# cg-saarland/hagrid

Hardware: AMD Instinct MI355X
Metric: Mrays/s (primary traversal) + grid build ms, 1M-tri scene @1/2/4/8 MI355X (higher is better)
Workload: dtype f32

## Files before the change

### hagrid_amd/csrc/ctx.h

```cpp
#pragma once

#include <hip/hip_runtime.h>

#include <atomic>
#include <cstdio>
#include <memory>
#include <string>
#include <unordered_map>
#include <vector>

#include "hagrid_amd.h"

namespace hagrid_impl {

struct Slot {
    void* ptr = nullptr;
    size_t size = 0;
    bool in_use = false;
    int refs = 0;
};

}

namespace hagrid_impl {

struct TravImageCache {
    void* table = nullptr;
    size_t table_bytes = 0;
    int wide_records = 0;
    void* blocks = nullptr;
    size_t block_bytes = 0;
    bool valid = false;
    bool uniform = false;
    bool general = false;
    int slim = 0;
    int vtop_k = 0;
    uint32_t vtop_base = 0;
    bool detached = false;
    bool borrowed = false;
    std::shared_ptr<std::atomic<bool>> alive;
    const void* entries = nullptr; const void* cells = nullptr; const void* refs = nullptr;
    int num_cells = 0, num_entries = 0, num_refs = 0, shift = 0, dims[3] = {0, 0, 0}, cell_bytes = 32;
    int max_ref = -1;
    void* alt_blocks = nullptr; void* alt_table = nullptr; size_t alt_block_bytes = 0, alt_table_bytes = 0; int alt_wide_records = 0, alt_slim = 0;
};

}

namespace hagrid_impl {
enum MailboxWord : int {
    kMbxRowLen = 300,
    kMbxOrderStale = 304,
    kMbxReadBackEpoch = 310,
    kMbxHeadSuggest = 312,
    kMbxPriorStats = 316,
};
enum ScratchWord : int {
    kScrRowLenBinned = 232,
    kScrRowLen = 236,
    kScrMaxRef = 240,
    kScrBlobFlag = 250,
};
}

struct hagrid_ctx {
    int device = 0;
    hipStream_t stream = nullptr;
    bool keep = false;
    int num_cus = 0;

    std::vector<hagrid_impl::Slot> slots;
    std::unordered_map<void*, int> tracker;
    size_t usage = 0, max_usage = 0;

    hipEvent_t ev_begin = nullptr, ev_end = nullptr;

    int* mailbox = nullptr;
    int* dscratch = nullptr;
    unsigned long long* lb_state = nullptr;
    size_t lb_words = 0;
    unsigned lb_epoch = 0;
    int* row_scores = nullptr;
    int* bin_diff = nullptr;

    int ray_binning = 0;
    int opt_variant = 0;
    int opt_lookback = 1;
    int opt_merge_inplace = 1;
    int opt_merge_inplace_iters = 0;
    int opt_merge_inplace_div = 0;
    int opt_merge_inplace_room = 0;
    int opt_merge_narrow = 1;
    int opt_expand_voxel_map = 1;
    int opt_expand_subset_only = 1;
    int opt_image_width = 0;
    int opt_band_rows = 0;
    int opt_super_log2 = 3;
    int opt_xcd_chunk_log2 = -2;
    int opt_narrow = 1;
    int opt_image_max_mb = 0;
    int opt_quad_head = 20;
    int opt_image_vtop = 1;
    int opt_image_uniform = 1;
    int opt_row_cache = 1;
    struct RayHints {
        const void* key_rays = nullptr; int key_n = 0;
        const void* rowlen_rays = nullptr; int rowlen_n = 0, rowlen_age = 0, rowlen_known = -1, rowlen_seen = 0; bool rows_from_origins = false ;
        hipEvent_t rowlen_evt = nullptr; bool rowlen_pending = false;
        int* lpt_buf = nullptr; int lpt_cap = 0; const void* lpt_rays = nullptr; int lpt_n = 0, lpt_blocks = 0, lpt_age = 0, lpt_period = 32, lpt_rot = 0 ; bool rot_adopted = false ;
        hipEvent_t trial_evt[2] = {nullptr, nullptr}; bool trial_pending = false, trial_with_head = false, head_disabled = false;
        float t_base = 0.0f, t_head = 0.0f; int n_base = 0, n_head = 0, trial_opt = -1 ; unsigned head_serial = 0 ; bool lpt_valid = false;
        int lpt_epoch = 1 , relearn_streak = 0, cooldown = 0, cooldown_len = 64; unsigned long long relearn_clock = 0;
        hipEvent_t share_evt[12][2] = {}; int share_issued = 0, share_done = 0, share_choice = -1 , share_ncand = 0 , share_shape_nc = 0 , share_cands[4] = {0, 0, 0, 0} ,
            share_last = -1 , share_launches = 0; float share_t[4] = {0.0f, 0.0f, 0.0f, 0.0f}; unsigned share_serial = 0 ;
        int trial_kind = 0 , n_all = 0, all_stage = 0 ; float t_all = 0.0f; bool learned_all = false;
        bool learned_once = false;
        unsigned order_serial = 0;
        bool cmp_pending = false, cmp_done = false; int n_conf = 0; float t_conf = 0.0f;
        bool order_loses = false;
        int last_report = -1;
        unsigned long long used = 0;
    };
    static constexpr int kRayHints = 4;
    RayHints hints[kRayHints];
    unsigned long long hint_clock = 0;
    int opt_mailbox = -1;
    int opt_tail = 1;
    int opt_lds_pad = 0;
    int opt_tail_dual = -1;
    int opt_share_trial = 1;
    int opt_order_gate = 1;
    int opt_tile_order = -1;
    int opt_quad_tail = -1;
    int opt_image_slim = 1;
    int opt_image_general = 1;
    int opt_image = 2;

    int opt_id_is_steps = 0;

    hagrid_impl::TravImageCache image;
    unsigned image_serial = 0;
    int readback_epoch = 0;
    int opt_fast_readback = 1;
    int build_arena_tris = 0;
    size_t build_arena_hint = 0;
    hagrid_build_counts counts = {};

    std::string err;
};

namespace hagrid_impl {

inline int fail(hagrid_ctx* ctx, int code, const char* file, int line, const char* msg) {
    if (ctx) {
        char buf[512];
        snprintf(buf, sizeof(buf), "%s(%d): %s", file, line, msg);
        ctx->err = buf;
    }
    return code;
}

#define HG_FAIL(ctx, code, msg) return ::hagrid_impl::fail((ctx), (code), __FILE__, __LINE__, (msg))
#define HG_HIP(ctx, call)                                                                         \
    do {                                                                                          \
        hipError_t e_ = (call);                                                                   \
        if (e_ != hipSuccess) return ::hagrid_impl::fail((ctx), HAGRID_EHIP, __FILE__, __LINE__, hipGetErrorString(e_)); \
    } while (0)
#define HG_TRY(expr)                                                                              \
    do {                                                                                          \
        int rc_ = (expr);                                                                         \
        if (rc_ < 0) return rc_;                                                                  \
    } while (0)

void debug_sync(hagrid_ctx* ctx, const char* file, int line);
#ifdef HAGRID_DEBUG_SYNC
#define HG_DBG(ctx) ::hagrid_impl::debug_sync((ctx), __FILE__, __LINE__)
#else
#define HG_DBG(ctx) do { } while (0)
#endif

template <typename T>
inline T* pool_alloc(hagrid_ctx* ctx, size_t n) {
    return static_cast<T*>(hagrid_mem_alloc(ctx, (n ? n : 1) * sizeof(T)));
}

template <typename T>
inline T* pool_try_alloc(hagrid_ctx* ctx, size_t n) {
    const std::string saved = ctx->err;
    T* p = pool_alloc<T>(ctx, n);
    if (!p) { (void)hipGetLastError(); ctx->err = saved; }
    return p;
}

struct PoolTemps {
    hagrid_ctx* ctx;
    std::vector<void*> ptrs;
    explicit PoolTemps(hagrid_ctx* c) : ctx(c) {}
    PoolTemps(const PoolTemps&) = delete;
    PoolTemps& operator=(const PoolTemps&) = delete;
    template <typename T> T* get(size_t n) { T* p = pool_alloc<T>(ctx, n); if (p) ptrs.push_back(p); return p; }
    void drop(void* p) { for (auto& q : ptrs) if (q == p && p) { hagrid_mem_free(ctx, p); q = nullptr; } }
    void* keep(void* p) { for (auto& q : ptrs) if (q == p) q = nullptr; return p; }
    ~PoolTemps() { for (void* p : ptrs) if (p) hagrid_mem_free(ctx, p); }
};

int pool_split(hagrid_ctx* ctx, void* base, void* const* parts, int n);

int read_back(hagrid_ctx* ctx, const void* dptr, void* hptr, size_t bytes);

inline int grid_blocks(long long n, int block) { return (int)((n + block - 1) / block); }

unsigned long long* lookback_state(hagrid_ctx* ctx, int tiles, int words_per_tile, unsigned* epoch);

int trav_image_build(hagrid_ctx* ctx, const hagrid_grid* grid);
void trav_image_drop(hagrid_ctx* ctx);
bool trav_image_matches(const hagrid_ctx* ctx, const hagrid_grid* grid);
bool trav_image_stale(const hagrid_ctx* ctx);
void trav_image_source_touched(hagrid_ctx* ctx, const void* ptr, size_t bytes);

}
```

### hagrid_amd/csrc/expand.hip

```cpp
#include "ctx.h"
#include "wave_prims.h"

#include "hagrid/grid.h"
#include "hagrid/prims.h"

using namespace hagrid;
using namespace hagrid_impl;

namespace {

struct ExpandK { ivec3 dims; ivec3 top; int shift; vec3 gmin, cell_size, grid_inv; const int* voxel_cells; };
constexpr int kChanged = 1 << 3;
struct CellRec { ivec3 lo; int begin; ivec3 hi; int end; };

__device__ __forceinline__ CellRec load_cell(const Cell* cells, int i) {
    const int4* p = reinterpret_cast<const int4*>(cells) + 2 * size_t(i);
    const int4 a = p[0], b = p[1];
    CellRec c; c.lo = ivec3(a.x, a.y, a.z); c.begin = a.w; c.hi = ivec3(b.x, b.y, b.z); c.end = b.w;
    return c;
}
__device__ __forceinline__ int comp(const ivec3& v, int axis) { return axis == 0 ? v.x : (axis == 1 ? v.y : v.z); }


__device__ __forceinline__ int lower_bound_in(const int* __restrict__ a, int n, int x) {
    int lo = 0, hi = n;
    while (lo < hi) {
        const int mid = (lo + hi) >> 1;
        if (a[mid] < x) lo = mid + 1; else hi = mid;
    }
    return lo;
}

__device__ __forceinline__ bool contains_all(const int* __restrict__ big, int nbig, const int* __restrict__ small, int nsmall) {
    if (nsmall > nbig) return false;
    if (nsmall == 0) return true;
    if (nbig <= 4) {
        const int b0 = big[0], b1 = nbig > 1 ? big[1] : -1, b2 = nbig > 2 ? big[2] : -1, b3 = nbig > 3 ? big[3] : -1;
        const int s0 = small[0], s1 = nsmall > 1 ? small[1] : s0, s2 = nsmall > 2 ? small[2] : s0, s3 = nsmall > 3 ? small[3] : s0;
        auto in_big = [&](int x) { return (x == b0) | (x == b1) | (x == b2) | (x == b3); };
        return in_big(s0) & in_big(s1) & in_big(s2) & in_big(s3);
    }
    for (int j = 0; j < nsmall; j++) {
        const int x = small[j], at = lower_bound_in(big, nbig, x);
        if (at == nbig || big[at] != x) return false;
    }
    return true;
}

__device__ __forceinline__ Tri load_tri(const float4* __restrict__ tris, int i) {
    const float4* p = tris + 3 * size_t(i);
    const float4 a = p[0], b = p[1], c = p[2];
    return Tri(vec3(a.x, a.y, a.z), a.w, vec3(b.x, b.y, b.z), b.w, vec3(c.x, c.y, c.z), c.w);
}

__global__ void __launch_bounds__(kBlock) fill_voxel_cells(ExpandK k, const Entry* __restrict__ entries, int* __restrict__ voxel_cells, int voxels) {
    const int v = blockIdx.x * kBlock + threadIdx.x;
    if (v >= voxels) return;
    const int s = k.shift, m = (1 << s) - 1, top = v >> (3 * s), local = v & ((1 << (3 * s)) - 1);
    const int tx = top % k.top.x, ty = (top / k.top.x) % k.top.y, tz = top / (k.top.x * k.top.y);
    const ivec3 at((tx << s) + (local & m), (ty << s) + ((local >> s) & m), (tz << s) + (local >> (2 * s)));
    voxel_cells[v] = int(lookup_entry(entries, s, k.top, at));
}
__device__ __forceinline__ int cell_of_voxel(const ExpandK& k, const Entry* __restrict__ entries, const ivec3& at) {
    if (!k.voxel_cells) return int(lookup_entry(entries, k.shift, k.top, at));
    const int s = k.shift, m = (1 << s) - 1;
    const int top = (at.x >> s) + k.top.x * ((at.y >> s) + k.top.y * (at.z >> s));
    return k.voxel_cells[(top << (3 * s)) + (at.x & m) + (((at.y & m) + ((at.z & m) << s)) << s)];
}

template <int AXIS>
__device__ __forceinline__ int room_before_prim(const ExpandK& k, const Tri& prim, const CellRec& cell, const BBox& cross, int room, bool UP) {
    constexpr int A1 = (AXIS + 1) % 3, A2 = (AXIS + 2) % 3;
    const BBox pb = prim.bbox();
    const bool overlaps = get<A1>(pb.min) <= get<A1>(cross.max) && get<A1>(pb.max) >= get<A1>(cross.min) &&
                          get<A2>(pb.min) <= get<A2>(cross.max) && get<A2>(pb.max) >= get<A2>(cross.min);
    if (!overlaps) return room;
    const int layer = int(((UP ? get<AXIS>(pb.min) : get<AXIS>(pb.max)) - get<AXIS>(k.gmin)) * get<AXIS>(k.grid_inv));
    const int free_layers = UP ? layer - comp(cell.hi, AXIS) : comp(cell.lo, AXIS) - layer - 1;
    return max(min(room, free_layers), 0);
}

template <int AXIS, bool SUBSET_ONLY>
__device__ __forceinline__ int face_growth(const ExpandK& k, const Entry* __restrict__ entries, const int* __restrict__ refs, const float4* __restrict__ tris,
                                           const Cell* __restrict__ cells, const CellRec& cell, bool UP, bool& again) {
    constexpr int A1 = (AXIS + 1) % 3, A2 = (AXIS + 2) % 3;
    const int face = UP ? comp(cell.hi, AXIS) : comp(cell.lo, AXIS);
    const int extent = comp(k.dims, AXIS);
    if (UP ? face >= extent : face <= 0) return 0;
    const int layer = UP ? face : face - 1;
    const int lo1 = comp(cell.lo, A1), hi1 = comp(cell.hi, A1), lo2 = comp(cell.lo, A2), hi2 = comp(cell.hi, A2);
    const int own = cell.end - cell.begin;
    int reach = extent, room = extent;
    int u = lo1, v = lo2, row_step = comp(k.dims, A2);
    for (;;) {
        const ivec3 at = AXIS == 0 ? ivec3(layer, u, v) : (AXIS == 1 ? ivec3(v, layer, u) : ivec3(u, v, layer));
        const CellRec nb = load_cell(cells, cell_of_voxel(k, entries, at));
        reach = min(reach, UP ? comp(nb.hi, AXIS) - face : face - comp(nb.lo, AXIS));
        room = min(room, reach);
        const int theirs = nb.end - nb.begin;
        if (SUBSET_ONLY) {
            if (!contains_all(refs + cell.begin, own, refs + nb.begin, theirs)) { room = 0; break; }
        } else if (theirs > 0) {
            const BBox cross(k.gmin + k.cell_size * vec3(cell.lo), k.gmin + k.cell_size * vec3(cell.hi));
            int mine = 0;
            for (int j = 0; j < theirs && room > 0; j++) {
                const int id = refs[nb.begin + j];
                while (mine < own && refs[cell.begin + mine] < id) mine++;
                if (mine < own && refs[cell.begin + mine] == id) continue;
                room = room_before_prim<AXIS>(k, load_tri(tris, id), cell, cross, room, UP);
            }
            if (room == 0) break;
        }
        row_step = min(row_step, comp(nb.hi, A2) - v);
        u = comp(nb.hi, A1);
        if (u >= hi1) {
            u = lo1; v += row_step; row_step = comp(k.dims, A2);
            if (v >= hi2) break;
        }
    }
    again |= room == reach;
    return UP ? room : -room;
}

template <int axis, bool SUBSET_ONLY, bool PAIRED>
__device__ __forceinline__ void grow_cell(const ExpandK& k, const Entry* __restrict__ entries, const int* __restrict__ refs, const float4* __restrict__ tris,
                                          const Cell* __restrict__ cells, Cell* __restrict__ new_cells, unsigned char* __restrict__ cell_flags, int id, int flags, bool up) {
    CellRec cell = load_cell(cells, id);
    bool flag = false;
    int ov1, ov2;
    if (PAIRED) {
        bool again = false;
        const int mine = face_growth<axis, SUBSET_ONLY>(k, entries, refs, tris, cells, cell, up, again);
        const int other = __shfl_xor(mine, 1, 64);
        flag = again | (__shfl_xor(int(again), 1, 64) != 0);
        if (up) return;
        ov1 = mine; ov2 = other;
    } else {
        ov1 = face_growth<axis, SUBSET_ONLY>(k, entries, refs, tris, cells, cell, false, flag);
        ov2 = face_growth<axis, SUBSET_ONLY>(k, entries, refs, tris, cells, cell, true, flag);
    }
    if (axis == 0) { cell.lo.x += ov1; cell.hi.x += ov2; }
    if (axis == 1) { cell.lo.y += ov1; cell.hi.y += ov2; }
    if (axis == 2) { cell.lo.z += ov1; cell.hi.z += ov2; }
    cell_flags[id] = (unsigned char)((flag ? 1 << axis : 0) | (flags & ~((1 << axis) | kChanged)) | ((ov1 | ov2) ? kChanged : 0));
    int4* out = reinterpret_cast<int4*>(new_cells) + 2 * size_t(id);
    out[0] = make_int4(cell.lo.x, cell.lo.y, cell.lo.z, cell.begin);
    out[1] = make_int4(cell.hi.x, cell.hi.y, cell.hi.z, cell.end);
}

template <int axis, bool SUBSET_ONLY>
__global__ void __launch_bounds__(kBlock) overlap_step(ExpandK k, const Entry* __restrict__ entries, const int* __restrict__ refs,
                                                       const float4* __restrict__ tris, const Cell* __restrict__ cells, Cell* __restrict__ new_cells,
                                                       unsigned char* __restrict__ cell_flags, int num_cells) {
    const int id = xcd_block(blockIdx.x, gridDim.x) * kBlock + threadIdx.x;
    if (id >= num_cells) return;
    const int flags = cell_flags[id];
    if ((flags & (1 << axis)) == 0) {
        const int4* p = reinterpret_cast<const int4*>(cells) + 2 * size_t(id);
        int4* out = reinterpret_cast<int4*>(new_cells) + 2 * size_t(id);
        const int4 a = p[0], b = p[1];
        out[0] = a; out[1] = b;
        if (flags & kChanged) cell_flags[id] = (unsigned char)(flags & ~kChanged);
        return;
    }
    grow_cell<axis, SUBSET_ONLY, false>(k, entries, refs, tris, cells, new_cells, cell_flags, id, flags, false);
}

constexpr int kSelectItems = 16;
constexpr int kSelectTile = kBlock * kSelectItems;

template <int axis>
__global__ void __launch_bounds__(kBlock) expand_select(const Cell* __restrict__ cells, Cell* __restrict__ new_cells, unsigned char* __restrict__ cell_flags,
                                                        int num_cells, int* __restrict__ list, int* __restrict__ count) {
    __shared__ int tile_list[kSelectTile];
    __shared__ int tile_count, tile_base;
    if (threadIdx.x == 0) tile_count = 0;
    __syncthreads();
    const int base = blockIdx.x * kSelectTile;
    int fl[kSelectItems];
    #pragma unroll
    for (int j = 0; j < kSelectItems; j++) {
        const int id = base + j * kBlock + threadIdx.x;
        fl[j] = id < num_cells ? cell_flags[id] : 0;
    }
    #pragma unroll
    for (int j = 0; j < kSelectItems; j++) {
        const int id = base + j * kBlock + threadIdx.x;
        const int flags = fl[j];
        const bool listed = (flags & (1 << axis)) != 0;
        const unsigned long long m = __ballot(listed);
        int wbase = 0;
        if (lane_id() == 0 && m) wbase = atomicAdd(&tile_count, __popcll(m));
        wbase = __shfl(wbase, 0, 64);
        if (listed) {
            tile_list[wbase + __popcll(m & ((1ull << lane_id()) - 1ull))] = id;
        } else if (flags & kChanged) {
            const int4* p = reinterpret_cast<const int4*>(cells) + 2 * size_t(id);
            int4* out = reinterpret_cast<int4*>(new_cells) + 2 * size_t(id);
            const int4 a = p[0], b = p[1];
            out[0] = a; out[1] = b;
            cell_flags[id] = (unsigned char)(flags & ~kChanged);
        }
    }
    __syncthreads();
    if (threadIdx.x == 0) tile_base = tile_count ? atomicAdd(count, tile_count) : 0;
    __syncthreads();
    for (int i = threadIdx.x; i < tile_count; i += kBlock) list[tile_base + i] = tile_list[i];
}

template <int axis, bool SUBSET_ONLY>
__global__ void __launch_bounds__(kBlock) expand_listed(ExpandK k, const Entry* __restrict__ entries, const int* __restrict__ refs,
                                                        const float4* __restrict__ tris, const Cell* __restrict__ cells, Cell* __restrict__ new_cells,
                                                        unsigned char* __restrict__ cell_flags, const int* __restrict__ list, const int* __restrict__ count) {
    const int n = *count, active = (2 * n + kBlock - 1) / kBlock;
    if (int(blockIdx.x) >= active) return;
    const int t = xcd_block(blockIdx.x, active) * kBlock + threadIdx.x;
    const int i = t >> 1;
    if (i >= n) return;
    const int id = list[i];
    grow_cell<axis, SUBSET_ONLY, true>(k, entries, refs, tris, cells, new_cells, cell_flags, id, cell_flags[id], (t & 1) != 0);
}

template <int axis, bool SUBSET_ONLY>
void listed_step(hipStream_t st, const ExpandK& k, const Entry* entries, const int* refs, const float4* tris, const Cell* cells, Cell* other,
                 unsigned char* flags, int n, int* list, int* count) {
    expand_select<axis><<<grid_blocks(n, kSelectTile), kBlock, 0, st>>>(cells, other, flags, n, list, count);
    expand_listed<axis, SUBSET_ONLY><<<grid_blocks(2ll * n, kBlock), kBlock, 0, st>>>(k, entries, refs, tris, cells, other, flags, list, count);
}

}

extern "C" int hagrid_expand_grid(hagrid_ctx* ctx, hagrid_grid* grid, const void* tris_v, int iters) {
    if (!ctx || !grid) return HAGRID_EINVAL;
    const bool subset_only = ctx->opt_expand_subset_only != 0;
    if (!subset_only && !tris_v && iters > 0) HG_FAIL(ctx, HAGRID_EINVAL, "expand_grid: the precise mode needs the triangles");
    const float4* tris = static_cast<const float4*>(tris_v);
    if (iters <= 0) return HAGRID_OK;
    if (!grid->cells || !grid->entries || !grid->ref_ids) HG_FAIL(ctx, HAGRID_EINVAL, "expand_grid: incomplete (or compressed) grid");
    trav_image_drop(ctx);
    HG_HIP(ctx, hipSetDevice(ctx->device));
    hipStream_t st = ctx->stream;
    ExpandK k;
    k.top = ivec3(grid->dims[0], grid->dims[1], grid->dims[2]);
    k.dims = k.top << grid->shift;
    k.shift = grid->shift;
    {
        const vec3 lo(grid->bbox_min[0], grid->bbox_min[1], grid->bbox_min[2]), ext = vec3(grid->bbox_max[0], grid->bbox_max[1], grid->bbox_max[2]) - lo;
        k.gmin = lo; k.cell_size = ext / vec3(k.dims); k.grid_inv = vec3(k.dims) / ext;
    }
    const int n = grid->num_cells;
    Cell* cells = static_cast<Cell*>(grid->cells);
    Cell* other = pool_alloc<Cell>(ctx, size_t(n));
    unsigned char* flags = pool_alloc<unsigned char>(ctx, size_t(n));
    if (!other || !flags) { hagrid_mem_free(ctx, other); hagrid_mem_free(ctx, flags); return HAGRID_ENOMEM; }
    (void)hipMemsetAsync(flags, 0xFF, size_t(n), st);
    const Entry* entries = static_cast<const Entry*>(grid->entries);
    const int* refs = static_cast<const int*>(grid->ref_ids);
    const int blocks = grid_blocks(n, kBlock);
    int* list = iters > 1 ? pool_try_alloc<int>(ctx, size_t(n)) : nullptr;
    const long long voxels = (long long)k.dims.x * k.dims.y * k.dims.z;
    int* voxel_cells = (ctx->opt_expand_voxel_map && voxels <= (1ll << 28)) ? pool_try_alloc<int>(ctx, size_t(voxels)) : nullptr;
    k.voxel_cells = voxel_cells;
    if (voxel_cells) { ExpandK kf = k; kf.voxel_cells = nullptr; fill_voxel_cells<<<grid_blocks(voxels, kBlock), kBlock, 0, st>>>(kf, entries, voxel_cells, int(voxels)); HG_DBG(ctx); }
    int* counts = ctx->dscratch + 160;
    const int max_listed = 48;
    if (list) (void)hipMemsetAsync(counts, 0, max_listed * sizeof(int), st);
    int listed = 0;
    for (int it = 0; it < iters; it++) {
        if (it > 0 && list && listed + 3 <= max_listed) {
            if (subset_only) {
                listed_step<0, true>(st, k, entries, refs, tris, cells, other, flags, n, list, counts + listed++); std::swap(cells, other);
                listed_step<1, true>(st, k, entries, refs, tris, cells, other, flags, n, list, counts + listed++); std::swap(cells, other);
                listed_step<2, true>(st, k, entries, refs, tris, cells, other, flags, n, list, counts + listed++); std::swap(cells, other);
            } else {
                listed_step<0, false>(st, k, entries, refs, tris, cells, other, flags, n, list, counts + listed++); std::swap(cells, other);
                listed_step<1, false>(st, k, entries, refs, tris, cells, other, flags, n, list, counts + listed++); std::swap(cells, other);
                listed_step<2, false>(st, k, entries, refs, tris, cells, other, flags, n, list, counts + listed++); std::swap(cells, other);
            }
            continue;
        }
        if (subset_only) {
            overlap_step<0, true><<<blocks, kBlock, 0, st>>>(k, entries, refs, tris, cells, other, flags, n); HG_DBG(ctx); std::swap(cells, other);
            overlap_step<1, true><<<blocks, kBlock, 0, st>>>(k, entries, refs, tris, cells, other, flags, n); HG_DBG(ctx); std::swap(cells, other);
            overlap_step<2, true><<<blocks, kBlock, 0, st>>>(k, entries, refs, tris, cells, other, flags, n); HG_DBG(ctx); std::swap(cells, other);
        } else {
            overlap_step<0, false><<<blocks, kBlock, 0, st>>>(k, entries, refs, tris, cells, other, flags, n); HG_DBG(ctx); std::swap(cells, other);
            overlap_step<1, false><<<blocks, kBlock, 0, st>>>(k, entries, refs, tris, cells, other, flags, n); HG_DBG(ctx); std::swap(cells, other);
            overlap_step<2, false><<<blocks, kBlock, 0, st>>>(k, entries, refs, tris, cells, other, flags, n); HG_DBG(ctx); std::swap(cells, other);
        }
    }
    hipError_t e = hipGetLastError();
    if (e == hipSuccess) e = hipStreamSynchronize(st);
    ctx->counts.expand_passes = 3 * iters; ctx->counts.expand_cells = n;
    hagrid_mem_free(ctx, flags);
    hagrid_mem_free(ctx, other);
    hagrid_mem_free(ctx, list);
    hagrid_mem_free(ctx, voxel_cells);
    grid->cells = cells;
    if (e != hipSuccess) HG_FAIL(ctx, HAGRID_EHIP, hipGetErrorString(e));
    return HAGRID_OK;
}
```

### hagrid_amd/csrc/kat/kat.hip

```cpp
#include "../trav_kernels.h"
#include "hagrid_amd_kat.h"

#include <cstring>

using namespace hagrid;
using namespace hagrid_impl;
using namespace hagrid_trav;


namespace {

__global__ void kat_prim_ray(const Tri* tris, const Ray* rays, const int* idx, int n, int* ret, int* hid, float* ht) {
    const int i = blockIdx.x * blockDim.x + threadIdx.x;
    if (i >= n) return;
    Hit h(-1, rays[i].tmax, 0, 0);
    ret[i] = intersect_prim_ray(tris[idx[i]], rays[i], idx[i], h) ? 1 : 0;
    hid[i] = h.id; ht[i] = h.t;
}
__global__ void kat_prim_ray_uvs(const Tri* tris, const Ray* rays, const int* idx, int n, int* ret, int* hid, float* ht, float* hu, float* hv) {
    const int i = blockIdx.x * blockDim.x + threadIdx.x;
    if (i >= n) return;
    Hit h(-1, rays[i].tmax, 0, 0);
    ret[i] = intersect_prim_ray_uvs(tris[idx[i]], rays[i], idx[i], h) ? 1 : 0;
    hid[i] = h.id; ht[i] = h.t; hu[i] = h.u; hv[i] = h.v;
// ... 95 lines not shown
                o[4 + j] = id == none ? ~0u : id;
                if (id != none) cnt++;
            }
            o[3] = cnt | (links ? 0x40000000u : 0u);
        }
        return;
    }
}

struct Staged {
    hagrid_ctx* ctx; void* d = nullptr; size_t bytes;
    Staged(hagrid_ctx* c, const void* h, size_t b) : ctx(c), bytes(b) {
        d = hagrid_mem_alloc(ctx, b);
        if (d && h) hagrid_mem_copy_h2d(ctx, d, h, b);
    }
    ~Staged() { hagrid_mem_free(ctx, d); }
    int fetch(void* h) { return hagrid_mem_copy_d2h(ctx, h, d, bytes); }
};

}

extern "C" int hagrid_kat_intersect_prim_ray(hagrid_ctx* ctx, const void* tris, const void* rays, const int32_t* tri_index,
                                             int n, int32_t* ret, int32_t* hit_id, float* hit_t) {
    if (!ctx || n <= 0) return HAGRID_EINVAL;
    int max_idx = 0;
    for (int i = 0; i < n; i++) max_idx = std::max(max_idx, tri_index[i]);
    Staged t(ctx, tris, size_t(max_idx + 1) * 48), r(ctx, rays, size_t(n) * 32), ix(ctx, tri_index, size_t(n) * 4);
    Staged o0(ctx, nullptr, size_t(n) * 4), o1(ctx, nullptr, size_t(n) * 4), o2(ctx, nullptr, size_t(n) * 4);
    kat_prim_ray<<<grid_blocks(n, 64), 64, 0, ctx->stream>>>((const Tri*)t.d, (const Ray*)r.d, (const int*)ix.d, n, (int*)o0.d, (int*)o1.d, (float*)o2.d); HG_DBG(ctx);
    HG_HIP(ctx, hipGetLastError());
    HG_TRY(o0.fetch(ret)); HG_TRY(o1.fetch(hit_id)); HG_TRY(o2.fetch(hit_t));
    return HAGRID_OK;
}

extern "C" int hagrid_kat_intersect_prim_ray_uvs(hagrid_ctx* ctx, const void* tris, const void* rays, const int32_t* tri_index,
                                                 int n, int32_t* ret, int32_t* hit_id, float* hit_t, float* hit_u, float* hit_v) {
    if (!ctx || n <= 0) return HAGRID_EINVAL;
    int max_idx = 0;
    for (int i = 0; i < n; i++) max_idx = std::max(max_idx, tri_index[i]);
    Staged t(ctx, tris, size_t(max_idx + 1) * 48), r(ctx, rays, size_t(n) * 32), ix(ctx, tri_index, size_t(n) * 4);
    Staged o0(ctx, nullptr, size_t(n) * 4), o1(ctx, nullptr, size_t(n) * 4), o2(ctx, nullptr, size_t(n) * 4), o3(ctx, nullptr, size_t(n) * 4), o4(ctx, nullptr, size_t(n) * 4);
    kat_prim_ray_uvs<<<grid_blocks(n, 64), 64, 0, ctx->stream>>>((const Tri*)t.d, (const Ray*)r.d, (const int*)ix.d, n, (int*)o0.d, (int*)o1.d, (float*)o2.d, (float*)o3.d, (float*)o4.d); HG_DBG(ctx);
    HG_HIP(ctx, hipGetLastError());
    HG_TRY(o0.fetch(ret)); HG_TRY(o1.fetch(hit_id)); HG_TRY(o2.fetch(hit_t)); HG_TRY(o3.fetch(hit_u)); HG_TRY(o4.fetch(hit_v));
    return HAGRID_OK;
}

extern "C" int hagrid_kat_intersect_prim_cell(hagrid_ctx* ctx, const void* tris, const void* boxes, const int32_t* tri_index, int n, int32_t* ret) {
    if (!ctx || n <= 0) return HAGRID_EINVAL;
    int max_idx = 0;
    for (int i = 0; i < n; i++) max_idx = std::max(max_idx, tri_index[i]);
    Staged t(ctx, tris, size_t(max_idx + 1) * 48), b(ctx, boxes, size_t(n) * 32), ix(ctx, tri_index, size_t(n) * 4), o(ctx, nullptr, size_t(n) * 4);
    kat_prim_cell<<<grid_blocks(n, 64), 64, 0, ctx->stream>>>((const Tri*)t.d, (const BBox*)b.d, (const int*)ix.d, n, (int*)o.d); HG_DBG(ctx);
    HG_HIP(ctx, hipGetLastError());
    return o.fetch(ret);
}

extern "C" int hagrid_kat_compute_range(hagrid_ctx* ctx, const int32_t* dims3, const void* grid_bb, const void* obj_bb, int n, int32_t* out6) {
    if (!ctx || n <= 0) return HAGRID_EINVAL;
    Staged d(ctx, dims3, size_t(n) * 12), g(ctx, grid_bb, size_t(n) * 32), ob(ctx, obj_bb, size_t(n) * 32), o(ctx, nullptr, size_t(n) * 24);
    kat_range<<<grid_blocks(n, 64), 64, 0, ctx->stream>>>((const int*)d.d, (const BBox*)g.d, (const BBox*)ob.d, n, (int*)o.d); HG_DBG(ctx);
    HG_HIP(ctx, hipGetLastError());
    return o.fetch(out6);
}

extern "C" int hagrid_kat_compute_grid_dims(hagrid_ctx* ctx, const void* bb, const int32_t* num_prims, const float* density, int n, int32_t* out3) {
    if (!ctx || n <= 0) return HAGRID_EINVAL;
    Staged b(ctx, bb, size_t(n) * 32), np(ctx, num_prims, size_t(n) * 4), de(ctx, density, size_t(n) * 4), o(ctx, nullptr, size_t(n) * 12);
    kat_grid_dims<<<grid_blocks(n, 64), 64, 0, ctx->stream>>>((const BBox*)b.d, (const int*)np.d, (const float*)de.d, n, (int*)o.d); HG_DBG(ctx);
    HG_HIP(ctx, hipGetLastError());
    return o.fetch(out3);
}

extern "C" int hagrid_kat_lookup_entry(hagrid_ctx* ctx, const uint32_t* entries, int num_entries, int shift, const int32_t* top_dims3,
                                       const int32_t* voxels3, int n, uint32_t* out) {
    if (!ctx || n <= 0 || num_entries <= 0) return HAGRID_EINVAL;
    Staged e(ctx, entries, size_t(num_entries) * 4), v(ctx, voxels3, size_t(n) * 12), o(ctx, nullptr, size_t(n) * 4);
    kat_lookup<<<grid_blocks(n, 64), 64, 0, ctx->stream>>>((const Entry*)e.d, shift, ivec3(top_dims3[0], top_dims3[1], top_dims3[2]), (const int*)v.d, n, (uint32_t*)o.d); HG_DBG(ctx);
    HG_HIP(ctx, hipGetLastError());
    return o.fetch(out);
}

extern "C" int hagrid_kat_detect_ray_rows(hagrid_ctx* ctx, const void* rays_dev, int num_rays, float bbox_diag, int32_t* row_len) {
    if (!ctx || !rays_dev || num_rays < 0 || !row_len) return HAGRID_EINVAL;
    int* d = ctx->dscratch + 232;
    TraverseArgs a;
    memset(&a, 0, sizeof(a));
    a.rays = static_cast<const float4*>(rays_dev);
    a.max_x = bbox_diag; a.min_x = 0.0f;
    launch_detect(ctx, a, num_rays, d, 65536);
    HG_HIP(ctx, hipGetLastError());
    HG_TRY(read_back(ctx, d, row_len, sizeof(int)));
    *row_len &= kRowLenMask;
    return HAGRID_OK;
}

extern "C" int hagrid_kat_tile_slots(hagrid_ctx* ctx, int num_rays, int row_len, int super_log2, int xcd_chunk_log2, int32_t* slots) {
    if (!ctx || num_rays <= 0 || !slots || super_log2 < 0 || (super_log2 & 0xff) > 8) return HAGRID_EINVAL;
    const int blocks = grid_blocks(num_rays, 64);
    TraverseArgs a;
    memset(&a, 0, sizeof(a));
    a.num_rays = num_rays; a.row_len_hint = row_len; a.super_log2 = super_log2 & 0xff; a.band_rows = super_log2 >> 8; a.xcd_chunk_log2 = xcd_chunk_log2;
    Staged o(ctx, nullptr, size_t(blocks) * 64 * 4);
    if (!o.d) return HAGRID_ENOMEM;
    kat_tile_slots<<<blocks, 64, 0, ctx->stream>>>(a, (int*)o.d); HG_DBG(ctx);
    HG_HIP(ctx, hipGetLastError());
    return o.fetch(slots);
}

extern "C" int hagrid_kat_image_records(hagrid_ctx* ctx, const hagrid_grid* grid, const int32_t* voxels3, int n, uint32_t* records8, int64_t* image_bytes) {
    if (!ctx || !grid || n < 0) return HAGRID_EINVAL;
    if (!trav_image_matches(ctx, grid)) HG_FAIL(ctx, HAGRID_EINVAL, "no traversal image for this grid");
    if (image_bytes) *image_bytes = (int64_t)ctx->image.block_bytes + (int64_t)ctx->image.table_bytes;
    if (n == 0) return HAGRID_OK;
    TraverseArgs a;
    HG_TRY(make_args(ctx, grid, nullptr, nullptr, nullptr, 0, a));
    image_args(ctx, a);
    Staged v(ctx, voxels3, size_t(n) * 12), o(ctx, nullptr, size_t(n) * 32);
    if (!v.d || !o.d) return HAGRID_ENOMEM;
    kat_image_records<<<grid_blocks(n, 64), 64, 0, ctx->stream>>>(a, (const int*)v.d, n, (uint32_t*)o.d, 1, ctx->image.slim, ctx->image.uniform ? 1 : 0, ctx->image.general ? 1 : 0); HG_DBG(ctx);
    HG_HIP(ctx, hipGetLastError());
    return o.fetch(records8);
}

extern "C" int hagrid_kat_traverse_timed(hagrid_ctx* ctx, const hagrid_grid* grid, const void* tris, const void* rays, void* hits, int num_rays,
                                         int row_len, int tail, unsigned long long* times_dev, const int* tile_order_dev) {
    if (!ctx || !grid || !times_dev || num_rays <= 0) return HAGRID_EINVAL;
    if (!trav_image_matches(ctx, grid) || !(ctx->image.uniform && ctx->image.slim == 20))
        HG_FAIL(ctx, HAGRID_EINVAL, "kat_traverse_timed: needs the table-free image with 20-bit slim records of this grid");
    TraverseArgs a;
    HG_TRY(make_args(ctx, grid, tris, rays, hits, num_rays, a));
    image_args(ctx, a);
    a.row_len_hint = row_len; a.wave_times = times_dev; a.tile_order = tile_order_dev;
    const int blocks = grid_blocks(num_rays, 64);
    if (tail) traverse_kernel_tail<20, true><<<blocks, 64, 0, ctx->stream>>>(a);
    else      traverse_kernel_img<0, 20, 0, true><<<blocks, 64, 0, ctx->stream>>>(a);
    HG_DBG(ctx);
    HG_HIP(ctx, hipGetLastError());
    return HAGRID_OK;
}

extern "C" int hagrid_kat_set_option(hagrid_ctx* ctx, const char* key, int value) {
    if (!ctx || !key) return HAGRID_EINVAL;
    struct { const char* name; int* dst; int lo, hi; } table[] = {
        {"traverse.variant", &ctx->opt_variant, 0, 4},              {"traverse.narrow", &ctx->opt_narrow, 0, 1},
        {"traverse.image_uniform", &ctx->opt_image_uniform, 0, 2},  {"traverse.image_slim", &ctx->opt_image_slim, 1, 2}, {"traverse.image_general", &ctx->opt_image_general, 0, 2}, {"traverse.image_vtop", &ctx->opt_image_vtop, 0, 1}, {"traverse.quad_head", &ctx->opt_quad_head, 0, 1000}, {"ctx.fast_readback", &ctx->opt_fast_readback, 0, 1},
        {"traverse.tail", &ctx->opt_tail, 0, 1},                    {"traverse.quad_tail", &ctx->opt_quad_tail, -1, 100},
        {"traverse.tail_dual", &ctx->opt_tail_dual, -1, 1},        
        {"traverse.super_tile", &ctx->opt_super_log2, 0, 8},        {"traverse.xcd_chunk", &ctx->opt_xcd_chunk_log2, -2, 16},
        {"traverse.row_cache", &ctx->opt_row_cache, 0, 1},          {"traverse.lds_pad", &ctx->opt_lds_pad, 0, 65536},
        {"merge.narrow_cells", &ctx->opt_merge_narrow, 0, 1},       {"scan.lookback", &ctx->opt_lookback, 1, 2},
        {"traverse.order_gate", &ctx->opt_order_gate, 0, 1}, {"traverse.share_trial", &ctx->opt_share_trial, 0, 1}, {"traverse.band_rows", &ctx->opt_band_rows, 0, 1 << 16}, {"traverse.mailbox", &ctx->opt_mailbox, -1, 1},
        {"merge.inplace", &ctx->opt_merge_inplace, 0, 1},           {"merge.inplace_iters", &ctx->opt_merge_inplace_iters, 0, 1 << 20}, {"merge.inplace_room", &ctx->opt_merge_inplace_room, 0, 0x7fffffff}, {"merge.inplace_div", &ctx->opt_merge_inplace_div, 0, 1 << 20},
        {"expand.voxel_map", &ctx->opt_expand_voxel_map, 0, 1},
    };
    for (auto& t : table)
        if (!strcmp(key, t.name)) {
            if (value < t.lo || value > t.hi || (t.dst == &ctx->opt_variant && value == 3)) HG_FAIL(ctx, HAGRID_EINVAL, "kat_set_option: value out of range");
            *t.dst = value;
            return HAGRID_OK;
        }
    return hagrid_set_option(ctx, key, value);
}

extern "C" int hagrid_kat_order_state(hagrid_ctx* ctx, const void* rays, int32_t* out12, float* ms2 ) {
    if (!ctx || !out12) return HAGRID_EINVAL;
    for (int i = 0; i < 12; i++) out12[i] = 0;
    out12[0] = -1;
    for (int i = 0; i < hagrid_ctx::kRayHints; i++) {
        const hagrid_ctx::RayHints& h = ctx->hints[i];
        if (h.key_rays != rays) continue;
        const int v[12] = {i, h.lpt_valid, h.cooldown > 0, h.lpt_rot, h.head_disabled, h.n_base, h.n_head, h.share_choice >= 0 ? h.share_cands[h.share_choice] : -1, h.share_done + 100 * h.share_issued + 10000 * int(h.order_loses), h.n_all + 10 * int(h.learned_all) + 100 * h.cooldown, __atomic_load_n(ctx->mailbox + kMbxHeadSuggest + i, __ATOMIC_RELAXED), h.share_launches};
        for (int k = 0; k < 12; k++) out12[k] = v[k];
        if (ms2) { ms2[0] = h.t_base; ms2[1] = h.t_head; ms2[2] = h.t_all; ms2[3] = h.share_choice >= 0 ? h.share_t[h.share_choice] : 0.0f; }
        return HAGRID_OK;
    }
    return HAGRID_OK;
}

extern "C" int hagrid_kat_forget_hints(hagrid_ctx* ctx) {
    if (!ctx) return HAGRID_EINVAL;
    for (auto& h : ctx->hints) { h.key_rays = nullptr; h.key_n = 0; h.used = 0; h.lpt_rays = nullptr; h.lpt_valid = false; h.rowlen_rays = nullptr; h.rowlen_seen = 0; h.share_ncand = 0; h.share_shape_nc = 0; h.share_choice = -1; }
    return HAGRID_OK;
}
```

Before: 7712.

## Use packed 16-byte narrow cell records with inline ref lists during grid expansion

```diff
diff --git a/hagrid_amd/csrc/ctx.h b/hagrid_amd/csrc/ctx.h
--- a/hagrid_amd/csrc/ctx.h
+++ b/hagrid_amd/csrc/ctx.h
@@ -92,6 +92,7 @@
     int opt_merge_inplace_room = 0;
     int opt_merge_narrow = 1;
     int opt_expand_voxel_map = 1;
+    int opt_expand_narrow = 1;
     int opt_expand_subset_only = 1;
     int opt_image_width = 0;
     int opt_band_rows = 0;
diff --git a/hagrid_amd/csrc/expand.hip b/hagrid_amd/csrc/expand.hip
--- a/hagrid_amd/csrc/expand.hip
+++ b/hagrid_amd/csrc/expand.hip
@@ -9,15 +9,56 @@
 
 namespace {
 
-struct ExpandK { ivec3 dims; ivec3 top; int shift; vec3 gmin, cell_size, grid_inv; const int* voxel_cells; };
+struct ExpandK {
+    ivec3 dims; ivec3 top; int shift; vec3 gmin, cell_size, grid_inv;
+    const int* voxel_cells;
+    const Cell* orig;
+    int subset_only;
+};
 constexpr int kChanged = 1 << 3;
+constexpr int kGrew = 1 << 4;
 struct CellRec { ivec3 lo; int begin; ivec3 hi; int end; };
 
-__device__ __forceinline__ CellRec load_cell(const Cell* cells, int i) {
-    const int4* p = reinterpret_cast<const int4*>(cells) + 2 * size_t(i);
-    const int4 a = p[0], b = p[1];
-    CellRec c; c.lo = ivec3(a.x, a.y, a.z); c.begin = a.w; c.hi = ivec3(b.x, b.y, b.z); c.end = b.w;
+constexpr int kListShift = 29;
+constexpr uint32_t kPayload = (1u << kListShift) - 1u;
+constexpr int kLong = 7;
+
+template <bool NARROW>
+__device__ __forceinline__ CellRec load_cell(const void* cells, int i) {
+    CellRec c;
+    if (NARROW) {
+        const uint4 v = reinterpret_cast<const uint4*>(cells)[i];
+        c.lo = ivec3(int(v.x & 0xffffu), int(v.x >> 16), int(v.y & 0xffffu));
+        c.hi = ivec3(int(v.y >> 16), int(v.z & 0xffffu), int(v.z >> 16));
+        c.begin = int(v.w); c.end = 0;
+    } else {
+        const int4* p = reinterpret_cast<const int4*>(cells) + 2 * size_t(i);
+        const int4 a = p[0], b = p[1];
+        c.lo = ivec3(a.x, a.y, a.z); c.begin = a.w; c.hi = ivec3(b.x, b.y, b.z); c.end = b.w;
+    }
     return c;
+}
+template <bool NARROW>
+__device__ __forceinline__ void store_cell(void* cells, int i, const CellRec& c) {
+    if (NARROW) {
+        reinterpret_cast<uint4*>(cells)[i] = make_uint4(uint32_t(c.lo.x) | uint32_t(c.lo.y) << 16, uint32_t(c.lo.z) | uint32_t(c.hi.x) << 16,
+                                                        uint32_t(c.hi.y) | uint32_t(c.hi.z) << 16, uint32_t(c.begin));
+    } else {
+        int4* out = reinterpret_cast<int4*>(cells) + 2 * size_t(i);
+        out[0] = make_int4(c.lo.x, c.lo.y, c.lo.z, c.begin);
+        out[1] = make_int4(c.hi.x, c.hi.y, c.hi.z, c.end);
+    }
+}
+template <bool NARROW>
+__device__ __forceinline__ void copy_cell(const void* cells, void* new_cells, int i) {
+    if (NARROW) {
+        reinterpret_cast<uint4*>(new_cells)[i] = reinterpret_cast<const uint4*>(cells)[i];
+    } else {
+        const int4* p = reinterpret_cast<const int4*>(cells) + 2 * size_t(i);
+        int4* out = reinterpret_cast<int4*>(new_cells) + 2 * size_t(i);
+        const int4 a = p[0], b = p[1];
+        out[0] = a; out[1] = b;
+    }
 }
 __device__ __forceinline__ int comp(const ivec3& v, int axis) { return axis == 0 ? v.x : (axis == 1 ? v.y : v.z); }
 
@@ -47,19 +88,59 @@
     return true;
 }
 
+struct ListRef { int n, at, one; };
+__device__ __forceinline__ ListRef list_of(const ExpandK& k, uint32_t word, int cell) {
+    const int count = int(word >> kListShift), pay = int(word & kPayload);
+    ListRef l; l.at = pay; l.one = pay;
+    l.n = count == kLong ? reinterpret_cast<const int*>(k.orig)[8 * size_t(cell) + 7] - pay : count;
+    return l;
+}
+
+struct OwnList {
+    int n, b0, b1, b2, b3; const int* p;
+    __device__ __forceinline__ bool has(int x) const {
+        if (n <= 4) return (x == b0) | (x == b1) | (x == b2) | (x == b3);
+        const int at = lower_bound_in(p, n, x);
+        return at < n && p[at] == x;
+    }
+};
+__device__ __forceinline__ OwnList own_list(const ExpandK& k, const int* __restrict__ refs, uint32_t word, int cell) {
+    const ListRef l = list_of(k, word, cell);
+    const bool inline_id = (word >> kListShift) == 1u;
+    const bool regs = !inline_id && l.n <= 4;
+    OwnList o; o.n = l.n; o.p = refs + l.at;
+    o.b0 = inline_id ? l.one : (regs && l.n > 0 ? o.p[0] : -1);
+    o.b1 = regs && l.n > 1 ? o.p[1] : -1; o.b2 = regs && l.n > 2 ? o.p[2] : -1; o.b3 = regs && l.n > 3 ? o.p[3] : -1;
+    return o;
+}
+__device__ __forceinline__ bool own_contains(const ExpandK& k, const int* __restrict__ refs, const OwnList& own, uint32_t word, int nb) {
+    const int count = int(word >> kListShift);
+    if (count == 0) return true;
+    if (own.n == 0) return false;
+    if (count == 1) return own.has(int(word & kPayload));
+    const ListRef l = list_of(k, word, nb);
+    if (l.n > own.n) return false;
+    const int* small = refs + l.at;
+    if (own.n <= 4) {
+        const int s0 = small[0], s1 = l.n > 1 ? small[1] : s0, s2 = l.n > 2 ? small[2] : s0, s3 = l.n > 3 ? small[3] : s0;
+        return own.has(s0) & own.has(s1) & own.has(s2) & own.has(s3);
+    }
+    for (int j = 0; j < l.n; j++)
+        if (!own.has(small[j])) return false;
+    return true;
+}
+
 __device__ __forceinline__ Tri load_tri(const float4* __restrict__ tris, int i) {
     const float4* p = tris + 3 * size_t(i);
     const float4 a = p[0], b = p[1], c = p[2];
     return Tri(vec3(a.x, a.y, a.z), a.w, vec3(b.x, b.y, b.z), b.w, vec3(c.x, c.y, c.z), c.w);
 }
 
-__global__ void __launch_bounds__(kBlock) fill_voxel_cells(ExpandK k, const Entry* __restrict__ entries, int* __restrict__ voxel_cells, int voxels) {
-    const int v = blockIdx.x * kBlock + threadIdx.x;
-    if (v >= voxels) return;
+__device__ __forceinline__ int voxel_cell(const ExpandK& k, const Entry* __restrict__ entries, int v) {
     const int s = k.shift, m = (1 << s) - 1, top = v >> (3 * s), local = v & ((1 << (3 * s)) - 1);
     const int tx = top % k.top.x, ty = (top / k.top.x) % k.top.y, tz = top / (k.top.x * k.top.y);
     const ivec3 at((tx << s) + (local & m), (ty << s) + ((local >> s) & m), (tz << s) + (local >> (2 * s)));
-    voxel_cells[v] = int(lookup_entry(entries, s, k.top, at));
+    return int(lookup_entry(entries, s, k.top, at));
 }
 __device__ __forceinline__ int cell_of_voxel(const ExpandK& k, const Entry* __restrict__ entries, const ivec3& at) {
     if (!k.voxel_cells) return int(lookup_entry(entries, k.shift, k.top, at));
@@ -80,10 +161,14 @@
     return max(min(room, free_layers), 0);
 }
 
-template <int AXIS, bool SUBSET_ONLY>
+template <int MODE> __device__ __forceinline__ bool subset_mode(const ExpandK& k) { return MODE == 0 ? k.subset_only != 0 : MODE == 1; }
+
+template <int AXIS, int MODE>
 __device__ __forceinline__ int face_growth(const ExpandK& k, const Entry* __restrict__ entries, const int* __restrict__ refs, const float4* __restrict__ tris,
-                                           const Cell* __restrict__ cells, const CellRec& cell, bool UP, bool& again) {
+                                           const void* __restrict__ cells, const CellRec& cell, const OwnList& mine_list, bool UP, bool& again) {
     constexpr int A1 = (AXIS + 1) % 3, A2 = (AXIS + 2) % 3;
+    constexpr bool NARROW = MODE != 0;
+    const bool subset_only = subset_mode<MODE>(k);
     const int face = UP ? comp(cell.hi, AXIS) : comp(cell.lo, AXIS);
     const int extent = comp(k.dims, AXIS);
     if (UP ? face >= extent : face <= 0) return 0;
@@ -94,13 +179,29 @@
     int u = lo1, v = lo2, row_step = comp(k.dims, A2);
     for (;;) {
         const ivec3 at = AXIS == 0 ? ivec3(layer, u, v) : (AXIS == 1 ? ivec3(v, layer, u) : ivec3(u, v, layer));
-        const CellRec nb = load_cell(cells, cell_of_voxel(k, entries, at));
+        const int nb_id = cell_of_voxel(k, entries, at);
+        const CellRec nb = load_cell<NARROW>(cells, nb_id);
         reach = min(reach, UP ? comp(nb.hi, AXIS) - face : face - comp(nb.lo, AXIS));
         room = min(room, reach);
-        const int theirs = nb.end - nb.begin;
-        if (SUBSET_ONLY) {
-            if (!contains_all(refs + cell.begin, own, refs + nb.begin, theirs)) { room = 0; break; }
-        } else if (theirs > 0) {
+        if (subset_only) {
+            const bool sub = NARROW ? own_contains(k, refs, mine_list, uint32_t(nb.begin), nb_id)
+                                    : contains_all(refs + cell.begin, own, refs + nb.begin, nb.end - nb.begin);
+            if (!sub) { room = 0; break; }
+        } else if (NARROW) {
+            const int count = int(uint32_t(nb.begin) >> kListShift);
+            if (count > 0) {
+                const ListRef l = list_of(k, uint32_t(nb.begin), nb_id);
+                const BBox cross(k.gmin + k.cell_size * vec3(cell.lo), k.gmin + k.cell_size * vec3(cell.hi));
+                for (int j = 0; j < l.n && room > 0; j++) {
+                    int id = l.one;
+                    if (count != 1) id = refs[l.at + j];
+                    if (mine_list.has(id)) continue;
+                    room = room_before_prim<AXIS>(k, load_tri(tris, id), cell, cross, room, UP);
+                }
+                if (room == 0) break;
+            }
+        } else if (nb.end - nb.begin > 0) {
+            const int theirs = nb.end - nb.begin;
             const BBox cross(k.gmin + k.cell_size * vec3(cell.lo), k.gmin + k.cell_size * vec3(cell.hi));
             int mine = 0;
             for (int j = 0; j < theirs && room > 0; j++) {
@@ -122,55 +223,53 @@
     return UP ? room : -room;
 }
 
-template <int axis, bool SUBSET_ONLY, bool PAIRED>
+template <int axis, int MODE, bool PAIRED>
 __device__ __forceinline__ void grow_cell(const ExpandK& k, const Entry* __restrict__ entries, const int* __restrict__ refs, const float4* __restrict__ tris,
-                                          const Cell* __restrict__ cells, Cell* __restrict__ new_cells, unsigned char* __restrict__ cell_flags, int id, int flags, bool up) {
-    CellRec cell = load_cell(cells, id);
+                                          const void* __restrict__ cells, void* __restrict__ new_cells, unsigned char* __restrict__ cell_flags, int id, int flags, bool up) {
+    constexpr bool NARROW = MODE != 0;
+    CellRec cell = load_cell<NARROW>(cells, id);
+    OwnList own = {};
+    if (NARROW) own = own_list(k, refs, uint32_t(cell.begin), id);
     bool flag = false;
     int ov1, ov2;
     if (PAIRED) {
         bool again = false;
-        const int mine = face_growth<axis, SUBSET_ONLY>(k, entries, refs, tris, cells, cell, up, again);
+        const int mine = face_growth<axis, MODE>(k, entries, refs, tris, cells, cell, own, up, again);
         const int other = __shfl_xor(mine, 1, 64);
         flag = again | (__shfl_xor(int(again), 1, 64) != 0);
         if (up) return;
         ov1 = mine; ov2 = other;
     } else {
-        ov1 = face_growth<axis, SUBSET_ONLY>(k, entries, refs, tris, cells, cell, false, flag);
-        ov2 = face_growth<axis, SUBSET_ONLY>(k, entries, refs, tris, cells, cell, true, flag);
+        ov1 = face_growth<axis, MODE>(k, entries, refs, tris, cells, cell, own, false, flag);
+        ov2 = face_growth<axis, MODE>(k, entries, refs, tris, cells, cell, own, true, flag);
     }
     if (axis == 0) { cell.lo.x += ov1; cell.hi.x += ov2; }
     if (axis == 1) { cell.lo.y += ov1; cell.hi.y += ov2; }
     if (axis == 2) { cell.lo.z += ov1; cell.hi.z += ov2; }
-    cell_flags[id] = (unsigned char)((flag ? 1 << axis : 0) | (flags & ~((1 << axis) | kChanged)) | ((ov1 | ov2) ? kChanged : 0));
-    int4* out = reinterpret_cast<int4*>(new_cells) + 2 * size_t(id);
-    out[0] = make_int4(cell.lo.x, cell.lo.y, cell.lo.z, cell.begin);
-    out[1] = make_int4(cell.hi.x, cell.hi.y, cell.hi.z, cell.end);
-}
-
-template <int axis, bool SUBSET_ONLY>
+    cell_flags[id] = (unsigned char)((flag ? 1 << axis : 0) | (flags & ~((1 << axis) | kChanged)) | ((ov1 | ov2) ? kChanged | kGrew : 0));
+    store_cell<NARROW>(new_cells, id, cell);
+}
+
+template <int axis, int MODE>
 __global__ void __launch_bounds__(kBlock) overlap_step(ExpandK k, const Entry* __restrict__ entries, const int* __restrict__ refs,
-                                                       const float4* __restrict__ tris, const Cell* __restrict__ cells, Cell* __restrict__ new_cells,
+                                                       const float4* __restrict__ tris, const void* __restrict__ cells, void* __restrict__ new_cells,
                                                        unsigned char* __restrict__ cell_flags, int num_cells) {
     const int id = xcd_block(blockIdx.x, gridDim.x) * kBlock + threadIdx.x;
     if (id >= num_cells) return;
     const int flags = cell_flags[id];
     if ((flags & (1 << axis)) == 0) {
-        const int4* p = reinterpret_cast<const int4*>(cells) + 2 * size_t(id);
-        int4* out = reinterpret_cast<int4*>(new_cells) + 2 * size_t(id);
-        const int4 a = p[0], b = p[1];
-        out[0] = a; out[1] = b;
+        copy_cell<MODE != 0>(cells, new_cells, id);
         if (flags & kChanged) cell_flags[id] = (unsigned char)(flags & ~kChanged);
         return;
     }
-    grow_cell<axis, SUBSET_ONLY, false>(k, entries, refs, tris, cells, new_cells, cell_flags, id, flags, false);
+    grow_cell<axis, MODE, false>(k, entries, refs, tris, cells, new_cells, cell_flags, id, flags, false);
 }
 
 constexpr int kSelectItems = 16;
 constexpr int kSelectTile = kBlock * kSelectItems;
 
-template <int axis>
-__global__ void __launch_bounds__(kBlock) expand_select(const Cell* __restrict__ cells, Cell* __restrict__ new_cells, unsigned char* __restrict__ cell_flags,
+template <bool NARROW>
+__global__ void __launch_bounds__(kBlock) expand_select(int axis, const void* __restrict__ cells, void* __restrict__ new_cells, unsigned char* __restrict__ cell_flags,
                                                         int num_cells, int* __restrict__ list, int* __restrict__ count) {
     __shared__ int tile_list[kSelectTile];
     __shared__ int tile_count, tile_base;
@@ -195,10 +294,7 @@
         if (listed) {
             tile_list[wbase + __popcll(m & ((1ull << lane_id()) - 1ull))] = id;
         } else if (flags & kChanged) {
-            const int4* p = reinterpret_cast<const int4*>(cells) + 2 * size_t(id);
-            int4* out = reinterpret_cast<int4*>(new_cells) + 2 * size_t(id);
-            const int4 a = p[0], b = p[1];
-            out[0] = a; out[1] = b;
+            copy_cell<NARROW>(cells, new_cells, id);
             cell_flags[id] = (unsigned char)(flags & ~kChanged);
         }
     }
@@ -208,9 +304,9 @@
     for (int i = threadIdx.x; i < tile_count; i += kBlock) list[tile_base + i] = tile_list[i];
 }
 
-template <int axis, bool SUBSET_ONLY>
+template <int axis, int MODE>
 __global__ void __launch_bounds__(kBlock) expand_listed(ExpandK k, const Entry* __restrict__ entries, const int* __restrict__ refs,
-                                                        const float4* __restrict__ tris, const Cell* __restrict__ cells, Cell* __restrict__ new_cells,
+                                                        const float4* __restrict__ tris, const void* __restrict__ cells, void* __restrict__ new_cells,
                                                         unsigned char* __restrict__ cell_flags, const int* __restrict__ list, const int* __restrict__ count) {
     const int n = *count, active = (2 * n + kBlock - 1) / kBlock;
     if (int(blockIdx.x) >= active) return;
@@ -218,14 +314,57 @@
     const int i = t >> 1;
     if (i >= n) return;
     const int id = list[i];
-    grow_cell<axis, SUBSET_ONLY, true>(k, entries, refs, tris, cells, new_cells, cell_flags, id, cell_flags[id], (t & 1) != 0);
-}
-
-template <int axis, bool SUBSET_ONLY>
-void listed_step(hipStream_t st, const ExpandK& k, const Entry* entries, const int* refs, const float4* tris, const Cell* cells, Cell* other,
+    grow_cell<axis, MODE, true>(k, entries, refs, tris, cells, new_cells, cell_flags, id, cell_flags[id], (t & 1) != 0);
+}
+
+__global__ void __launch_bounds__(kBlock) expand_prepare(ExpandK k, const Entry* __restrict__ entries, int* __restrict__ voxel_cells, int voxels,
+                                                         const Cell* __restrict__ cells, const int* __restrict__ refs, void* __restrict__ recs, int num_cells) {
+    const int t = blockIdx.x * kBlock + threadIdx.x;
+    if (voxel_cells && t < voxels) voxel_cells[t] = voxel_cell(k, entries, t);
+    if (recs && t < num_cells) {
+        CellRec c = load_cell<false>(cells, t);
+        const int n = c.end - c.begin;
+        uint32_t word = uint32_t(min(n, kLong)) << kListShift | uint32_t(c.begin);
+        if (n == 0) word = 0u;
+        if (n == 1) {
+            const uint32_t id = uint32_t(refs[c.begin]);
+            if (id <= kPayload) word = 1u << kListShift | id;
+            else word = uint32_t(kLong) << kListShift | uint32_t(c.begin);
+        }
+        c.begin = int(word);
+        store_cell<true>(recs, t, c);
+    }
+}
+__global__ void __launch_bounds__(kBlock) expand_write_back(const void* __restrict__ recs, const unsigned char* __restrict__ cell_flags, Cell* __restrict__ cells, int num_cells) {
+    const int t = blockIdx.x * kBlock + threadIdx.x;
+    if (t >= num_cells || !(cell_flags[t] & kGrew)) return;
+    const CellRec c = load_cell<true>(recs, t);
+    int* out = reinterpret_cast<int*>(cells) + 8 * size_t(t);
+    out[0] = c.lo.x; out[1] = c.lo.y; out[2] = c.lo.z;
+    out[4] = c.hi.x; out[5] = c.hi.y; out[6] = c.hi.z;
+}
+
+template <int axis, int MODE>
+void listed_step(hipStream_t st, const ExpandK& k, const Entry* entries, const int* refs, const float4* tris, const void* cells, void* other,
                  unsigned char* flags, int n, int* list, int* count) {
-    expand_select<axis><<<grid_blocks(n, kSelectTile), kBlock, 0, st>>>(cells, other, flags, n, list, count);
-    expand_listed<axis, SUBSET_ONLY><<<grid_blocks(2ll * n, kBlock), kBlock, 0, st>>>(k, entries, refs, tris, cells, other, flags, list, count);
+    expand_select<MODE != 0><<<grid_blocks(n, kSelectTile), kBlock, 0, st>>>(axis, cells, other, flags, n, list, count);
+    expand_listed<axis, MODE><<<grid_blocks(2ll * n, kBlock), kBlock, 0, st>>>(k, entries, refs, tris, cells, other, flags, list, count);
+}
+
+template <int MODE>
+void expansion_iter(hagrid_ctx* ctx, const ExpandK& k, const Entry* entries, const int* refs, const float4* tris, void*& cells, void*& other,
+                    unsigned char* flags, int n, int* list, int* counts) {
+    hipStream_t st = ctx->stream;
+    if (counts) {
+        listed_step<0, MODE>(st, k, entries, refs, tris, cells, other, flags, n, list, counts + 0); std::swap(cells, other);
+        listed_step<1, MODE>(st, k, entries, refs, tris, cells, other, flags, n, list, counts + 1); std::swap(cells, other);
+        listed_step<2, MODE>(st, k, entries, refs, tris, cells, other, flags, n, list, counts + 2); std::swap(cells, other);
+        return;
+    }
+    const int blocks = grid_blocks(n, kBlock);
+    overlap_step<0, MODE><<<blocks, kBlock, 0, st>>>(k, entries, refs, tris, cells, other, flags, n); HG_DBG(ctx); std::swap(cells, other);
+    overlap_step<1, MODE><<<blocks, kBlock, 0, st>>>(k, entries, refs, tris, cells, other, flags, n); HG_DBG(ctx); std::swap(cells, other);
+    overlap_step<2, MODE><<<blocks, kBlock, 0, st>>>(k, entries, refs, tris, cells, other, flags, n); HG_DBG(ctx); std::swap(cells, other);
 }
 
 }
@@ -250,53 +389,46 @@
     }
     const int n = grid->num_cells;
     Cell* cells = static_cast<Cell*>(grid->cells);
-    Cell* other = pool_alloc<Cell>(ctx, size_t(n));
+    k.orig = cells;
+    k.subset_only = subset_only;
+    const bool narrow = ctx->opt_expand_narrow && std::max(k.dims.x, std::max(k.dims.y, k.dims.z)) < 65536 && (long long)grid->num_refs <= (long long)kPayload;
+    void* work = narrow ? static_cast<void*>(pool_alloc<uint4>(ctx, 2 * size_t(n))) : static_cast<void*>(pool_alloc<Cell>(ctx, size_t(n)));
     unsigned char* flags = pool_alloc<unsigned char>(ctx, size_t(n));
-    if (!other || !flags) { hagrid_mem_free(ctx, other); hagrid_mem_free(ctx, flags); return HAGRID_ENOMEM; }
-    (void)hipMemsetAsync(flags, 0xFF, size_t(n), st);
+    if (!work || !flags) { hagrid_mem_free(ctx, work); hagrid_mem_free(ctx, flags); return HAGRID_ENOMEM; }
+    void* cur = narrow ? work : static_cast<void*>(cells);
+    void* other = narrow ? static_cast<void*>(static_cast<uint4*>(work) + n) : work;
+    (void)hipMemsetAsync(flags, 0x07 | kChanged, size_t(n), st);
     const Entry* entries = static_cast<const Entry*>(grid->entries);
     const int* refs = static_cast<const int*>(grid->ref_ids);
-    const int blocks = grid_blocks(n, kBlock);
     int* list = iters > 1 ? pool_try_alloc<int>(ctx, size_t(n)) : nullptr;
     const long long voxels = (long long)k.dims.x * k.dims.y * k.dims.z;
     int* voxel_cells = (ctx->opt_expand_voxel_map && voxels <= (1ll << 28)) ? pool_try_alloc<int>(ctx, size_t(voxels)) : nullptr;
     k.voxel_cells = voxel_cells;
-    if (voxel_cells) { ExpandK kf = k; kf.voxel_cells = nullptr; fill_voxel_cells<<<grid_blocks(voxels, kBlock), kBlock, 0, st>>>(kf, entries, voxel_cells, int(voxels)); HG_DBG(ctx); }
+    {
+        const long long threads = std::max(voxel_cells ? voxels : 0ll, narrow ? (long long)n : 0ll);
+        ExpandK kf = k; kf.voxel_cells = nullptr;
+        if (threads > 0) { expand_prepare<<<grid_blocks(threads, kBlock), kBlock, 0, st>>>(kf, entries, voxel_cells, int(voxels), cells, refs, narrow ? cur : nullptr, n); HG_DBG(ctx); }
+    }
     int* counts = ctx->dscratch + 160;
     const int max_listed = 48;
     if (list) (void)hipMemsetAsync(counts, 0, max_listed * sizeof(int), st);
     int listed = 0;
     for (int it = 0; it < iters; it++) {
-        if (it > 0 && list && listed + 3 <= max_listed) {
-            if (subset_only) {
-                listed_step<0, true>(st, k, entries, refs, tris, cells, other, flags, n, list, counts + listed++); std::swap(cells, other);
-                listed_step<1, true>(st, k, entries, refs, tris, cells, other, flags, n, list, counts + listed++); std::swap(cells, other);
-                listed_step<2, true>(st, k, entries, refs, tris, cells, other, flags, n, list, counts + listed++); std::swap(cells, other);
-            } else {
-                listed_step<0, false>(st, k, entries, refs, tris, cells, other, flags, n, list, counts + listed++); std::swap(cells, other);
-                listed_step<1, false>(st, k, entries, refs, tris, cells, other, flags, n, list, counts + listed++); std::swap(cells, other);
-                listed_step<2, false>(st, k, entries, refs, tris, cells, other, flags, n, list, counts + listed++); std::swap(cells, other);
-            }
-            continue;
-        }
-        if (subset_only) {
-            overlap_step<0, true><<<blocks, kBlock, 0, st>>>(k, entries, refs, tris, cells, other, flags, n); HG_DBG(ctx); std::swap(cells, other);
-            overlap_step<1, true><<<blocks, kBlock, 0, st>>>(k, entries, refs, tris, cells, other, flags, n); HG_DBG(ctx); std::swap(cells, other);
-            overlap_step<2, true><<<blocks, kBlock, 0, st>>>(k, entries, refs, tris, cells, other, flags, n); HG_DBG(ctx); std::swap(cells, other);
-        } else {
-            overlap_step<0, false><<<blocks, kBlock, 0, st>>>(k, entries, refs, tris, cells, other, flags, n); HG_DBG(ctx); std::swap(cells, other);
-            overlap_step<1, false><<<blocks, kBlock, 0, st>>>(k, entries, refs, tris, cells, other, flags, n); HG_DBG(ctx); std::swap(cells, other);
-            overlap_step<2, false><<<blocks, kBlock, 0, st>>>(k, entries, refs, tris, cells, other, flags, n); HG_DBG(ctx); std::swap(cells, other);
-        }
-    }
+        int* cnt = nullptr;
+        if (it > 0 && list && listed + 3 <= max_listed) { cnt = counts + listed; listed += 3; }
+        if (!narrow) expansion_iter<0>(ctx, k, entries, refs, tris, cur, other, flags, n, list, cnt);
+        else if (subset_only) expansion_iter<1>(ctx, k, entries, refs, tris, cur, other, flags, n, list, cnt);
+        else expansion_iter<2>(ctx, k, entries, refs, tris, cur, other, flags, n, list, cnt);
+    }
+    if (narrow && n > 0) { expand_write_back<<<grid_blocks(n, kBlock), kBlock, 0, st>>>(cur, flags, cells, n); HG_DBG(ctx); }
     hipError_t e = hipGetLastError();
     if (e == hipSuccess) e = hipStreamSynchronize(st);
     ctx->counts.expand_passes = 3 * iters; ctx->counts.expand_cells = n;
     hagrid_mem_free(ctx, flags);
-    hagrid_mem_free(ctx, other);
+    hagrid_mem_free(ctx, narrow ? work : other);
     hagrid_mem_free(ctx, list);
     hagrid_mem_free(ctx, voxel_cells);
-    grid->cells = cells;
+    if (!narrow) grid->cells = cur;
     if (e != hipSuccess) HG_FAIL(ctx, HAGRID_EHIP, hipGetErrorString(e));
     return HAGRID_OK;
 }
diff --git a/hagrid_amd/csrc/kat/kat.hip b/hagrid_amd/csrc/kat/kat.hip
--- a/hagrid_amd/csrc/kat/kat.hip
+++ b/hagrid_amd/csrc/kat/kat.hip
@@ -271,7 +271,7 @@
         {"merge.narrow_cells", &ctx->opt_merge_narrow, 0, 1},       {"scan.lookback", &ctx->opt_lookback, 1, 2},
         {"traverse.order_gate", &ctx->opt_order_gate, 0, 1}, {"traverse.share_trial", &ctx->opt_share_trial, 0, 1}, {"traverse.band_rows", &ctx->opt_band_rows, 0, 1 << 16}, {"traverse.mailbox", &ctx->opt_mailbox, -1, 1},
         {"merge.inplace", &ctx->opt_merge_inplace, 0, 1},           {"merge.inplace_iters", &ctx->opt_merge_inplace_iters, 0, 1 << 20}, {"merge.inplace_room", &ctx->opt_merge_inplace_room, 0, 0x7fffffff}, {"merge.inplace_div", &ctx->opt_merge_inplace_div, 0, 1 << 20},
-        {"expand.voxel_map", &ctx->opt_expand_voxel_map, 0, 1},
+        {"expand.voxel_map", &ctx->opt_expand_voxel_map, 0, 1},     {"expand.narrow", &ctx->opt_expand_narrow, 0, 1},
     };
     for (auto& t : table)
         if (!strcmp(key, t.name)) {
```

Result: no change. 7710 (median of 2 runs) (-0.0%).
